# claforte/RayTracingWeekend.jl

Hardware: AMD Instinct MI355X
Metric: Msamples/s (pixels x spp) on scene_random_spheres 1920x1080 (higher is better)
Workload: dtype f32

## Files before the change

raytracingweekend.jl_amd/csrc/rtw_abi.hip:

```cpp
#include "rtw_host.hpp"
#include "rtw_kernels.hpp"

namespace rtwh {

__thread char g_err[512] = "";

bool test_aids() {
    static const bool on = [] { const char *e = getenv("RTW_ENABLE_TEST_AIDS"); return e != nullptr && atoi(e) != 0; }();
    return on;
}
const char *aid_env(const char *name) { return test_aids() ? getenv(name) : nullptr; }
bool aid_flag(const char *name) { const char *e = aid_env(name); return e != nullptr && atoi(e) != 0; }

int fail(int code, const char *fmt, ...) {
    va_list ap;
    va_start(ap, fmt);
    vsnprintf(g_err, sizeof g_err, fmt, ap);
    va_end(ap);
    return code;
}

std::mutex g_mu;
std::vector<CtxPtr> g_ctx;
std::atomic<unsigned> g_generation{1};
// ... 159 lines not shown
    *count = n;
    return 0;
}

const char *rtw_last_error(void) { return g_err; }

int rtw_scene_upload_f32(const rtw_scene_f32 *s, int device, rtw_scene_handle *out) { return upload_scene_f32(s, device, out); }
int rtw_scene_upload_f64(const rtw_scene_f64 *s, int device, rtw_scene_handle *out) { return upload_scene_f64(s, device, out); }

int rtw_scene_free(rtw_scene_handle h) {
    if (!h) return 0;
    DeviceGuard guard;
    HIP_IGNORE(hipSetDevice(h->device));
    void *ptrs[] = {h->geom, h->mat0, h->mat1, h->scan, h->mf_ops, h->c_mf_ops, h->c_mf_box, h->c_bound, h->c_exact, h->c_mat0, h->c_mat1, h->c_orig};
    for (void *q : ptrs) if (q) HIP_IGNORE(hipFree(q));
    delete h;
    return 0;
}

int rtw_render_device_f32(rtw_scene_handle s, const rtw_camera_f32 *c, const rtw_params *p, void *d_out, void *stream) {
    return render_device(s, c, p, d_out, stream);
}
int rtw_render_device_f64(rtw_scene_handle s, const rtw_camera_f64 *c, const rtw_params *p, void *d_out, void *stream) {
    return render_device(s, c, p, d_out, stream);
}
int rtw_render_f32(const rtw_scene_f32 *s, const rtw_camera_f32 *c, const rtw_params *p, float *out) {
    return render_host_f32(s, c, p, out);
}
int rtw_render_f64(const rtw_scene_f64 *s, const rtw_camera_f64 *c, const rtw_params *p, double *out) {
    return render_host_f64(s, c, p, out);
// ... 73 lines not shown
```

raytracingweekend.jl_amd/csrc/rtw_host.hpp:

```cpp
#pragma once
#pragma GCC visibility push(default)
#include "../../include/rtw_hip.h"
#pragma GCC visibility pop

#include <hip/hip_runtime.h>

#include <algorithm>
#include <atomic>
#include <cmath>
#include <cstdarg>
#include <cstdio>
#include <cstdlib>
#include <cstring>
#include <map>
#include <memory>
#include <mutex>
#include <string>
#include <thread>
#include <type_traits>
#include <vector>

#pragma GCC visibility push(hidden)

namespace rtw { struct DevCounters; }


struct rtw_scene_dev {
    int device;
    int is_f64;
    int n, n_pad;
    void *geom, *mat0, *mat1;
    void *scan;
    void *mf_ops;
    int mf_blocks;
    float mf_sc, mf_sigma2, mf_oo_keep, mf_o1_coef, mf_o_max;
    int n_huge, huge[2];
    void *c_mf_ops, *c_mf_box;
    float c_glo[3], c_ghi[3];
    int c_mf_blocks;
    float c_grid[6];
    int c_n_inlane, c_inlane[8];
    void *c_bound, *c_exact, *c_mat0, *c_mat1;
    unsigned short *c_orig;
    int c_groups_pad, c_big;
    double c_cs[3], c_rs;
    uint64_t content_hash;
};

namespace rtwh {

extern __thread char g_err[512];
// ... 146 lines not shown
```

raytracingweekend.jl_amd/csrc/rtw_kernels.hpp:

```cpp
#pragma once
#include "rtw_device.hpp"

namespace rtw {

#define RTW_JOB_PX 16
#ifndef RTW_SLOT_BYTES
#define RTW_SLOT_BYTES 4608
#endif
#define RTW_REF_BITS 9
#define RTW_REF_MASK 511u
#define RTW_SLOT_FREE 0xffffffffu
#define RTW_SLOT_OPENING 0xfffffffeu
#define RTW_SLOT_OPENING_BIT 0x80000000u
#define RTW_JOB_EOF 0xffffffffu
#define RTW_JOB_RETRY 0xfffffffeu

struct KParams {
    int width, height, spp, max_depth;
    uint64_t seed;
    int n_chunks;
    int chunk_spp;
    int shard_index, shard_count;
    int tiles_i, tiles_j;
    unsigned total_jobs;
// ... 345 lines not shown
    WgShared<T> *sh = reinterpret_cast<WgShared<T> *>(smem + list_bytes);
    constexpr size_t cell_bytes = MFMA ? mfma_cell_bytes<T>() : 0;
    V4 *lds_geom = reinterpret_cast<V4 *>(smem + list_bytes + shared_bytes + cell_bytes);
    WaveScratch ws = {nullptr, nullptr, nullptr};
    [[maybe_unused]] ulonglong2 *pool_rng = nullptr;
    [[maybe_unused]] unsigned long long pool_valid = 0;
    if constexpr (MFMA) {
        static_assert(list_bytes == 4 * RTW_PAIR_CAP * sizeof(unsigned), "the pair lists reuse the per-lane list area");
        const unsigned wv = threadIdx.x >> 6;
        unsigned char *cells = smem + list_bytes + shared_bytes;
        ws.pairs = reinterpret_cast<unsigned *>(smem) + wv * RTW_PAIR_CAP;
        ws.keys = reinterpret_cast<unsigned long long *>(cells) + wv * 64;
        ws.kidx = reinterpret_cast<unsigned *>(cells + 4 * 64 * sizeof(unsigned long long)) + wv * 64;
        pool_rng = reinterpret_cast<ulonglong2 *>(cells + mfma_cell_bytes<T>() - 4 * 64 * 16) + wv * 64;
    }
    unsigned short *lds_orig = reinterpret_cast<unsigned short *>(lds_geom + (CULL ? cull_exact_count(cull) : 0));
    [[maybe_unused]] unsigned *lds_tab = reinterpret_cast<unsigned *>(reinterpret_cast<unsigned char *>(lds_orig) + (CULL ? ((size_t)cull_exact_count(cull) * sizeof(unsigned short) + 15) / 16 * 16 : 0));
    if (threadIdx.x < P_arg.n_slots) { JobSlot *S0 = sh->slot(threadIdx.x, P_arg.slot_stride); S0->ready_seq = RTW_SLOT_FREE; S0->job = 0u; }
    if (threadIdx.x == 0) { sh->ticket = 0u; sh->eof = 0u; sh->fin_waves = 0u; sh->fin_segments = 0ull; sh->fin_samples = 0ull; sh->jobs.jc = 0ull; sh->jobs.jc_lock = 0u; sh->jobs.queue_off = 0u; sh->jobs.last_g = 0u; sh->jobs.static_used = 0u; sh->cam = cam_arg; sh->P = P_arg; }
    const KParams &P = sh->P;
    if (LDS_SCENE) {
        if (CULL) stage_cull_scene<T>(cull, lds_geom, lds_orig);
        else stage_scene<T>(scene, lds_geom);
        if constexpr (CULL && MFMA) {
            const unsigned *gt = reinterpret_cast<const unsigned *>(cull.mf_box + 8 * (cull.mf_blocks + 1));
            for (int i = threadIdx.x; i < cull_tab_words(cull.mf_blocks); i += blockDim.x) lds_tab[i] = gt[i];
        }
    }
    __syncthreads();

    if (lane == 0 && (threadIdx.x >> 6) < 4u) sh->t_wave[threadIdx.x >> 6] = wall_clock64();
    unsigned pool_next = 0, pool_end = 0;
    unsigned pool_slot = 0, pool_b = 0;
    bool have_ticket = false;
    unsigned tk_seq = 0, tk_b = 0;

    unsigned long long n_segments = 0, n_samples = 0;

// ... 12 lines not shown

    PhaseClock<PROFILE> clk;
    for (;;) {
        clk.start();
        T t_hit = 0;
        int idx = -1;
        if constexpr (MFMA && CULL) {
            if (__any(has_ray)) {
                MfmaCull mc = mfma_cull_of(cull);
                if (LDS_SCENE) mc.tab = lds_tab;
                if (LDS_SCENE) idx = hit_world_mfma<T>(scene, (const V4 *)lds_geom, ro, rd, has_ray, (T)1e-4, t_hit, ws, lane, clk, &mc, (const unsigned short *)lds_orig);
                else idx = hit_world_mfma<T>(scene, cull.exact, ro, rd, has_ray, (T)1e-4, t_hit, ws, lane, clk, &mc, cull.orig);
            }
        } else if constexpr (MFMA) {
            if (__any(has_ray)) {
                if (LDS_SCENE) idx = hit_world_mfma<T>(scene, (const V4 *)lds_geom, ro, rd, has_ray, (T)1e-4, t_hit, ws, lane, clk);
                else idx = hit_world_mfma<T>(scene, scene.geom, ro, rd, has_ray, (T)1e-4, t_hit, ws, lane, clk);
            }
        } else if (has_ray) {
            if (CULL && LDS_SCENE)
                idx = hit_world_cull<T, 256>(cull, (const V4 *)lds_geom, (const unsigned short *)lds_orig, ro, rd, (T)1e-4,
                                             (T)__builtin_huge_val(), t_hit, my_list, clk);
            else if (CULL)
                idx = hit_world_cull<T, 256>(cull, cull.exact, cull.orig, ro, rd, (T)1e-4, (T)__builtin_huge_val(), t_hit, my_list, clk);
            else if (LDS_SCENE)
                idx = hit_world<T, 256>(scene, (const V4 *)lds_geom, ro, rd, (T)1e-4, (T)__builtin_huge_val(), t_hit, my_list, clk);
            else
                idx = hit_world<T, 256>(scene, scene.geom, ro, rd, (T)1e-4, (T)__builtin_huge_val(), t_hit, my_list, clk);
        }
        n_segments += (unsigned long long)__popcll(__ballot(has_ray));
        clk.lap(2);
        if (PROFILE) { clk.count(8, 1u); clk.count(9, (unsigned)__popcll(__ballot(has_ray))); if (!__any(has_ray)) clk.count(10, 1u); }
// ... 311 lines not shown
```

raytracingweekend.jl_amd/csrc/rtw_launch.hip:

```cpp
#include "rtw_scene_view.hpp"
#include "rtw_kernels.hpp"
#include "rtw_instances.hpp"
#ifdef RTW_WITH_POOL
#include "rtw_pool.hpp"
#endif

namespace rtwh {

void make_udiv(unsigned d, unsigned *m, unsigned *s) {
    if (d <= 1) { *m = 0; *s = 0x80000000u; return; }
    unsigned l = 0;
    while ((1ull << l) < d) ++l;
    *m = (unsigned)((((1ull << l) - d) << 32) / d + 1);
    *s = l - 1;
}

template <typename T, typename CamT>
int launch_render(rtw_scene_handle scene, const CamT *cam, int n_views, const uint64_t *seeds, const rtw_params *p, void *d_out, hipStream_t stream,
                  RenderRec **rec_out, CtxPtr *ctx_out, const AccumPass *pass = nullptr) {
    if (!scene || !cam || (!d_out && !pass)) return fail(-1, "null argument");
    if (scene->is_f64 != (sizeof(T) == 8)) return fail(-4, "scene handle precision does not match the call");
    int nch, cs;
    if (int rc = validate_params(p, &nch, &cs)) return rc;
    if (pass) nch = pass->chunk_count;
// ... 43 lines not shown
    S.numerics = (p->flags & RTW_FLAG_NUMERICS_CONTRACT) ? rtw::NUM_CONTRACT : (p->flags & RTW_FLAG_NUMERICS_REFERENCE_FMA2) ? rtw::NUM_REFERENCE_FMA2 : rtw::NUM_REFERENCE;

    static const bool phase_profile = aid_env("RTW_PHASE_PROFILE") != nullptr;
    const size_t list_bytes = (size_t)RTW_LIST_CAP * 256 * sizeof(unsigned short);
    const size_t shared_bytes = (sizeof(rtw::WgShared<T>) + 15) / 16 * 16;
    const bool cull = (p->flags & RTW_FLAG_GROUP_CULL) != 0;
    rtw::CullScene<T> CS = cull_scene_of<T>(scene);
    CS.numerics = S.numerics;
    const size_t n_cull = (size_t)rtw::cull_exact_count(CS);
    static const bool force_valu = aid_env("RTW_SCAN") != nullptr && strcmp(aid_env("RTW_SCAN"), "valu") == 0;
    const bool mfma = (cull ? scene->c_mf_ops != nullptr : scene->mf_ops != nullptr) && !force_valu && !(p->flags & RTW_FLAG_SCAN_VALU);
    const size_t geom_bytes = cull ? n_cull * sizeof(V4) + ((n_cull * sizeof(unsigned short) + 15) / 16) * 16 +
                                         (mfma ? (size_t)rtw::cull_tab_words(scene->c_mf_blocks) * sizeof(unsigned) : 0)
                                   : (size_t)rtw::scene_geom_alloc(scene->n, scene->n_pad) * sizeof(V4);
    const bool lds_scene = geom_bytes <= RTW_LDS_SCENE_MAX_BYTES;
    const size_t lds_bytes = list_bytes + shared_bytes + (mfma ? rtw::mfma_cell_bytes<T>() : 0) + (lds_scene ? geom_bytes : 0);
    typedef void (*kern_t)(rtw::KParams, rtw::Camera<T>, rtw::DevScene<T>, rtw::CullScene<T>, T *, rtw::DevCounters *, rtw::BatchArgs<T>, rtw::AccumArgs);
    kern_t kern;
    if (cull && mfma && phase_profile) kern = lds_scene ? (kern_t)rtw::trace_kernel<T, true, true, true, true> : (kern_t)rtw::trace_kernel<T, false, false, true, true>;
    else if (cull && mfma) kern = lds_scene ? (kern_t)rtw::trace_kernel<T, false, true, true, true> : (kern_t)rtw::trace_kernel<T, false, false, true, true>;
    else if (cull && phase_profile) kern = lds_scene ? (kern_t)rtw::trace_kernel<T, true, true, true> : (kern_t)rtw::trace_kernel<T, false, false, true>;
    else if (cull) kern = lds_scene ? (kern_t)rtw::trace_kernel<T, false, true, true> : (kern_t)rtw::trace_kernel<T, false, false, true>;
    else if (mfma && phase_profile) kern = lds_scene ? (kern_t)rtw::trace_kernel<T, true, true, false, true> : (kern_t)rtw::trace_kernel<T, true, false, false, true>;
    else if (mfma) kern = lds_scene ? (kern_t)rtw::trace_kernel<T, false, true, false, true> : (kern_t)rtw::trace_kernel<T, false, false, false, true>;
    else if (phase_profile) kern = lds_scene ? (kern_t)rtw::trace_kernel<T, true, true, false> : (kern_t)rtw::trace_kernel<T, true, false, false>;
    else kern = lds_scene ? (kern_t)rtw::trace_kernel<T, false, true, false> : (kern_t)rtw::trace_kernel<T, false, false, false>;
    if (S.numerics == rtw::NUM_REFERENCE && lds_scene && mfma && !phase_profile)
        kern = cull ? (kern_t)rtw::trace_kernel<T, false, true, true, true, rtw::NUM_REFERENCE> : (kern_t)rtw::trace_kernel<T, false, true, false, true, rtw::NUM_REFERENCE>;
    const bool fixed = S.numerics == rtw::NUM_REFERENCE;
    if (batch && pass) kern = (kern_t)(sizeof(T) == 8 ? batch_accum_kernel_f64(cull, mfma, lds_scene, fixed, pass->adapt) : batch_accum_kernel_f32(cull, mfma, lds_scene, fixed, pass->adapt));
    else if (batch) kern = (kern_t)trace_instance_of<T, true, false, false>(cull, mfma, lds_scene, fixed);
// ... 101 lines not shown
        if (pass) {
            rtw::AccumView *hv = reinterpret_cast<rtw::AccumView *>(static_cast<char *>(rec->h_views) + cam_bytes + seed_bytes);
            for (int v = 0; v < n_views; ++v) { hv[v].words = pass->views[v].words; hv[v].samples = pass->views[v].samples; hv[v].pad = 0; }
            A.views = reinterpret_cast<const rtw::AccumView *>(static_cast<const char *>(rec->d_views) + cam_bytes + seed_bytes);
        }
        HIP_TRY(hipMemcpyAsync(rec->d_views, rec->h_views, bytes, hipMemcpyHostToDevice, stream));
        B.cams = reinterpret_cast<const rtw::Camera<T> *>(rec->d_views);
        B.seeds = reinterpret_cast<const unsigned long long *>(static_cast<const char *>(rec->d_views) + cam_bytes);
    }
    if (K.out_layout == 0 && p->shard_count > 1 && d_out)
        HIP_TRY(hipMemsetAsync(d_out, 0, (size_t)p->width * p->height * 3 * sizeof(T), stream));
    HIP_TRY(hipEventRecord(rec->ev0, stream));
    if (total_jobs > 0) {
        (void)hipGetLastError();
#ifdef RTW_WITH_POOL
        if (pool) hipLaunchKernelGGL(pool_kern, dim3((unsigned)grid), dim3((unsigned)block_threads), pool_lds, stream, K, C, S, (T *)d_out, rec->ctr);
        else
#endif
        hipLaunchKernelGGL(kern, dim3((unsigned)grid), dim3(256), lds_bytes, stream, K, C, S, CS, (T *)d_out, rec->ctr, B, A);
        HIP_TRY(hipGetLastError());
    }
    HIP_TRY(hipEventRecord(rec->ev1, stream));
    HIP_TRY(hipMemcpyAsync(rec->h_ctr, rec->ctr, rec->ctr_bytes, hipMemcpyDeviceToHost, stream));
    HIP_TRY(hipEventRecord(rec->ev2, stream));
    rec->used = true; rec->done = false;
    return 0;
}

int resolve_rec(RenderRec *r, rtw_stats_t *agg) {
    HIP_TRY(hipSetDevice(r->device));
    HIP_TRY(hipEventSynchronize(r->ev2));
// ... 82 lines not shown
```

raytracingweekend.jl_amd/csrc/rtw_scan.hpp:

```cpp
#pragma once
#include "rtw_path.hpp"

namespace rtw {

#define RTW_SPHERE_WORD 32
#define RTW_SPHERE_TAIL 8
__host__ __device__ inline int scene_geom_alloc(int n, int n_pad) {
    const int a = n_pad + RTW_SPHERE_TAIL, b = ((n + 31) / 32) * 32;
    return a > b ? a : b;
}
template <typename T> struct DevScene {
    const float *scan;
    const typename Vec4<T>::type *geom;
    const typename Vec4<T>::type *mat0;
    const typename Vec4<T>::type *mat1;
    int n, n_pad;
    const uint4 *mf_ops;
    int mf_blocks;
    float mf_sc;
    float mf_sigma2;
    float mf_oo_keep;
    float mf_o1_coef;
    float mf_o_max;
    int n_huge, huge[2];
    int numerics;
};

#define RTW_LIST_CAP 16
#define RTW_LDS_SCENE_MAX_BYTES (24 * 1024)

__device__ __forceinline__ uint32_t sign_word(float x) { return __float_as_uint(x); }
__device__ __forceinline__ uint32_t sign_word(double x) { return (uint32_t)((uint64_t)__double_as_longlong(x) >> 32); }

#ifndef RTW_SCAN_PRIO
#define RTW_SCAN_PRIO 1
#endif
template <typename T> struct ScanGroup;
template <> struct ScanGroup<float> { static constexpr int N = 4; };
template <> struct ScanGroup<double> { static constexpr int N = 4; };

// ... 164 lines not shown
```

raytracingweekend.jl_amd/csrc/rtw_scan_mfma.hpp:

```cpp
#pragma once
#include "rtw_scan.hpp"
#include "rtw_cull_tables.hpp"
#include "rtw_probes.hpp"

namespace rtw {

#define RTW_PAIR_CAP 512
typedef _Float16 rtw_h8 __attribute__((ext_vector_type(8)));
typedef float rtw_f16v __attribute__((ext_vector_type(16)));

__host__ __device__ inline int cull_tab_words(int blocks) { return ((blocks + 31) / 32 > 0 ? (blocks + 31) / 32 : 1) * RTW_CULL_TAB_WORDS; }
struct CullGrid {
    float inv[3], off[3];
};

struct MfmaCull {
    const uint4 *ops;
    const float *box;
    int blocks;
    float cs[3], rs;
    const void *mat0;
    float glo[3], ghi[3];
    int n_huge;
    int n_exact;
// ... 102 lines not shown
            }
            total += (unsigned)__popcll(act);
        }
    }
    __builtin_amdgcn_wave_barrier();
    test_singles<T, WITH_R>(num, src, rad, o, d, tmin, ws, singles, total, lane, orig, prof, sink);
    __builtin_amdgcn_wave_barrier();
}

template <typename T, typename SRC, typename RAD, typename ORIG = NoOrig, typename SINK = NoSink>
__device__ __forceinline__ void resolve_pairs(int num, SRC src, RAD rad, V3<T> o, V3<T> d, T tmin, const WaveScratch &ws, unsigned n, unsigned lane, ORIG orig = ORIG(), unsigned *prof = nullptr, SINK sink = SINK()) {
    if (num == NUM_REFERENCE_FMA2) resolve_pairs_impl<T, true>(num, src, rad(), o, d, tmin, ws, n, lane, orig, prof, sink);
    else resolve_pairs_impl<T, false>(num, src, nullptr, o, d, tmin, ws, n, lane, orig, prof, sink);
}

template <typename T, typename SRC, typename ORIG = NoOrig, typename CLK = NoClock, typename SINK = NoSink>
__device__ __forceinline__ int hit_world_mfma(const DevScene<T> &w, SRC src, V3<T> o, V3<T> d, bool has_ray, T tmin, T &t_hit,
                                              const WaveScratch &ws, unsigned lane, CLK &&clk = NoClock(),
                                              const MfmaCull *mc = nullptr, ORIG orig = ORIG(), SINK sink = SINK()) {
    constexpr bool CULLED = !__is_same(ORIG, NoOrig);
    auto rad = [&]() -> const typename Vec4<T>::type * { if constexpr (CULLED) return (const typename Vec4<T>::type *)mc->mat0; else return w.mat0; };
    const float ox = (float)o.x, oy = (float)o.y, oz = (float)o.z, dx = (float)d.x, dy = (float)d.y, dz = (float)d.z;
    const float s2 = __builtin_fmaf(dz, dz, __builtin_fmaf(dy, dy, dx * dx));
    const float oinf = __builtin_fmaxf(__builtin_fmaxf(__builtin_fabsf(ox), __builtin_fabsf(oy)), __builtin_fabsf(oz));
    const bool ok = has_ray && s2 <= 1.0009f && oinf <= w.mf_o_max;
    if constexpr (SINK::on()) { if (has_ray) sink.ray(lane, ok, w.mf_sc); }
    const float q = __builtin_fmaf(oz, dz, __builtin_fmaf(oy, dy, ox * dx));
    const float oo = __builtin_fmaf(oz, oz, __builtin_fmaf(oy, oy, ox * ox));
    const float o1 = (__builtin_fabsf(ox) + __builtin_fabsf(oy)) + __builtin_fabsf(oz);
    const float oop = __builtin_fmaf(oo, w.mf_oo_keep, -(w.mf_o1_coef * o1));
    const float tq = w.mf_sigma2 * __builtin_fmaf(q, q, -oop);
    const float z = ok ? 1.0f : 0.0f, z2 = z + z, zs2 = z2 * w.mf_sc;
    const float fp[3] = {__builtin_fmaf(-q, dx, ox) * zs2, __builtin_fmaf(-q, dy, oy) * zs2, __builtin_fmaf(-q, dz, oz) * zs2};
    const float dx2 = dx * z2, dy2 = dy * z2, dz2 = dz * z2;
    const float fq[6] = {dx2 * dx, dy2 * dy, dz2 * dz, (dx2 + dx2) * dy, (dx2 + dx2) * dz, (dy2 + dy2) * dz};
// ... 80 lines not shown
        B1[0] = __builtin_bit_cast(rtw_h8, q10); B1[1] = __builtin_bit_cast(rtw_h8, q11);
        B2[0] = __builtin_bit_cast(rtw_h8, q20); B2[1] = __builtin_bit_cast(rtw_h8, q21);
    }
    const unsigned lane_const = lane << 16;
    unsigned total = 0;
    {
        unsigned long long key0 = ~0ull;
        [[maybe_unused]] unsigned kidx0 = 0u;
        using V4 = typename Vec4<T>::type;
        const int n_huge = CULLED ? (RTW_INLANE_FILTER ? mc->n_exact : mc->n_huge) : w.n_huge;
        for (int hgi = 0; hgi < n_huge; ++hgi) {
            int si;
            if constexpr (CULLED) si = __builtin_amdgcn_readfirstlane((int)mc->tab[6 * RTW_CULL_BINS + 4 + hgi]);
            else si = hgi == 0 ? w.huge[0] : w.huge[1];
            const V4 sg = src[si];
            if constexpr (SINK::on()) { if (has_ray) { if constexpr (CULLED) sink.inlane(lane, (int)orig[si]); else sink.inlane(lane, si); } }
            T hb_, disc_, root_ = 0;
            T rr_ = T(0);
            if (w.numerics == NUM_REFERENCE_FMA2) rr_ = rad()[si].x;
            sphere_disc<T>(w.numerics, sg.x, sg.y, sg.z, sg.w, rr_, o, d, hb_, disc_);
            if (has_ray && sphere_root<T>(hb_, disc_, tmin, (T)__builtin_huge_val(), root_)) {
                unsigned tie = (unsigned)si;
                if constexpr (CULLED) tie = ((unsigned)orig[si] << 16) | (unsigned)si;
                if constexpr (sizeof(T) == 4) {
                    const unsigned low = CULLED ? ((0xffffu - (tie >> 16)) << 16) | (tie & 0xffffu) : 0xffffffffu - tie;
                    const unsigned long long k = ((unsigned long long)__float_as_uint((float)root_) << 32) | (unsigned long long)low;
                    key0 = k < key0 ? k : key0;
                } else {
                    const unsigned long long tb = (unsigned long long)__double_as_longlong((double)root_);
                    if (tb < key0 || (tb == key0 && tie + 1u > kidx0)) { key0 = tb; kidx0 = tie + 1u; }
                }
            }
        }
        if constexpr (sizeof(T) == 4) ws.keys[lane] = key0;
        else { ws.keys[lane] = key0; ws.kidx[lane] = kidx0; }
    }
    if constexpr (CULLED && RTW_INLANE_FILTER) {
        using V4 = typename Vec4<T>::type;
        for (int hgi = mc->n_exact; hgi < mc->n_huge; ++hgi) {
            const int si = __builtin_amdgcn_readfirstlane((int)mc->tab[6 * RTW_CULL_BINS + 4 + hgi]);
// ... 124 lines not shown
        if (m != 0u) {
            const unsigned pos = __builtin_amdgcn_mbcnt_hi((unsigned)(act >> 32), __builtin_amdgcn_mbcnt_lo((unsigned)act, total));
            reinterpret_cast<uint2 *>(ws.pairs)[pos] = uint2{m, lane_const + (unsigned)cur * 32u};
        }
        total += (unsigned)__popcll(act);
        clk.lap(4);
    }
    }
    if (use_prio) __builtin_amdgcn_s_setprio(sizeof(T) == 4 ? 1 : 0);
    { unsigned pr[3] = {0u, 0u, 0u}; resolve_pairs<T>(w.numerics, src, rad, o, d, tmin, ws, total, lane, orig, clk.on() ? pr : nullptr, sink); clk.count(13, total); clk.count(14, pr[0]); clk.count(15, pr[1]); clk.count(28, pr[2]); }
    RTW_PROBE_RESOLVE_TWICE();
    clk.lap(5);
    int idx;
    if constexpr (sizeof(T) == 4) {
        const unsigned long long k = ws.keys[lane];
        idx = k == ~0ull ? -1 : (CULLED ? (int)((unsigned)k & 0xffffu) : (int)(0xffffffffu - (unsigned)k));
        t_hit = __uint_as_float((unsigned)(k >> 32));
    } else {
        const unsigned long long k = ws.keys[lane];
        const unsigned ki = ws.kidx[lane];
        idx = ki == 0u ? -1 : (CULLED ? (int)((ki - 1u) & 0xffffu) : (int)ki - 1);
        t_hit = __longlong_as_double((long long)k);
    }
    if (!has_ray) idx = -1;
    return idx;
}

}
```

raytracingweekend.jl_amd/csrc/rtw_scene.hip:

```cpp
#include "rtw_scene_view.hpp"
#include "rtw_cull_tables.hpp"

namespace rtwh {

template <typename SceneT>
void kd_split(const SceneT *s, std::vector<int> &ids, int lo, int hi, std::vector<std::vector<int>> &groups) {
    const int cnt = hi - lo;
    if (cnt <= RTW_CULL_GS) {
        if (cnt > 0) groups.emplace_back(ids.begin() + lo, ids.begin() + hi);
        return;
    }
    double mn[3] = {1e300, 1e300, 1e300}, mx[3] = {-1e300, -1e300, -1e300};
    for (int k = lo; k < hi; ++k) {
        const double c[3] = {(double)s->cx[ids[k]], (double)s->cy[ids[k]], (double)s->cz[ids[k]]};
        for (int a = 0; a < 3; ++a) { mn[a] = std::min(mn[a], c[a]); mx[a] = std::max(mx[a], c[a]); }
    }
    int ax = 0;
    for (int a = 1; a < 3; ++a) if (mx[a] - mn[a] > mx[ax] - mn[ax]) ax = a;
    const int unit = cnt > 2 * RTW_CULL_GS ? 2 * RTW_CULL_GS : RTW_CULL_GS;
    int half = ((cnt / 2 + unit - 1) / unit) * unit;
    if (half >= cnt) half = cnt - 1;
    auto key = [&](int i) { return ax == 0 ? (double)s->cx[i] : ax == 1 ? (double)s->cy[i] : (double)s->cz[i]; };
    std::nth_element(ids.begin() + lo, ids.begin() + lo + half, ids.begin() + hi, [&](int a, int b) { return key(a) < key(b); });
    kd_split(s, ids, lo, lo + half, groups);
    kd_split(s, ids, lo + half, hi, groups);
}

template <typename T, typename V4, typename SceneT>
void material_rows(const SceneT *s, int i, V4 &m0, V4 &m1) {
    m0 = V4{s->r[i], s->param[i], (T)s->kind[i], (T)0};
    m1 = V4{s->ar[i], s->ag[i], s->ab[i], (T)0};
    if (s->kind[i] == rtw::DIELECTRIC) {
        const rtw::DielConst<T> c = rtw::dielectric_constants<T>(s->param[i]);
        m0.w = c.inv_ir;
        m1 = V4{c.r0_front, c.r0_back, (T)0, (T)0};
    }
}

template <typename T, typename V4>
int build_mfma_operands(const std::vector<V4> &geom, int n, rtw_scene_dev *h, void **ops_out, int *blocks_out, int n_skip = 0, const int *skip = nullptr);

template <typename T, typename SceneT>
int build_cull(const SceneT *s, rtw_scene_dev *h) {
    using V4 = typename rtw::Vec4<T>::type;
    const int n = s->n;
    constexpr int pair = 2 * RTW_CULL_BG, GS = RTW_CULL_GS;
    std::vector<int> small_ids, big_ids;
    if (n > 0) {
        std::vector<double> rr(n);
        for (int i = 0; i < n; ++i) rr[i] = std::fabs((double)s->r[i]);
        std::vector<double> tmp(rr);
        std::nth_element(tmp.begin(), tmp.begin() + (n - 1) / 2, tmp.end());
        const double thr = 4.0 * tmp[(n - 1) / 2];
        for (int i = 0; i < n; ++i) (rr[i] > thr ? big_ids : small_ids).push_back(i);
    }
// ... 110 lines not shown
            for (int a = 0; a < 3; ++a) { h->c_glo[a] = std::min(h->c_glo[a], q[a]); h->c_ghi[a] = std::max(h->c_ghi[a], q[4 + a]); }
        }
        CullTables ct;
        build_cull_tables(bx.data(), nb, h->c_glo, h->c_ghi, h->c_n_inlane, h->c_inlane, &ct);
        for (int k = 0; k < 3; ++k) { h->c_grid[k] = ct.inv[k]; h->c_grid[3 + k] = ct.off[k]; }
        std::vector<float> cells(ct.words.size(), 0.0f);
        memcpy(cells.data(), ct.words.data(), ct.words.size() * sizeof(unsigned));
        bx.insert(bx.end(), cells.begin(), cells.end());
        HIP_TRY(hipMalloc(&h->c_mf_box, bx.size() * sizeof(float)));
        HIP_TRY(hipMemcpy(h->c_mf_box, bx.data(), bx.size() * sizeof(float), hipMemcpyHostToDevice));
    }
    return 0;
}

template <typename T, typename V4>
int build_mfma_operands(const std::vector<V4> &geom, int n, rtw_scene_dev *h, void **ops_out, int *blocks_out, int n_skip, const int *skip) {
    *ops_out = nullptr; *blocks_out = 0;
    if (n <= 0) return 0;
    auto live = [&](int i) { return i < n && (double)geom[i].w > -1e29; };
    auto in_filter = [&](int i) { if (!live(i)) return false; for (int k = 0; k < n_skip; ++k) if (skip[k] == i) return false; return true; };
    double emax = 0;
    for (int i = 0; i < n; ++i) {
        if (!live(i)) continue;
        const double r = std::sqrt(std::fabs((double)geom[i].w));
        emax = std::max(emax, std::max(std::max(std::fabs((double)(float)geom[i].x), std::fabs((double)(float)geom[i].y)),
                                       std::max(std::fabs((double)(float)geom[i].z), r)));
    }
    if (!(emax > 0) || !std::isfinite(emax)) return 0;
    int ex = 0;
    (void)std::frexp(emax, &ex);
    if (ex > 40 || ex < -40) return 0;
    const double sc = std::ldexp(1.0, 8 - ex), sig2 = sc * sc;
    const double phi_c = std::ldexp(1.0, -25) / sc, phi_k = std::ldexp(1.0, -20) / sig2;
    const double A_S = std::ldexp(1.0, -17), A_r = std::ldexp(12.0, -22);
    auto split = [](double x, unsigned &p1, unsigned &p2) {
        const float xf = (float)x;
        const _Float16 h1 = (_Float16)xf;
        const _Float16 h2 = (_Float16)(xf - (float)h1);
        unsigned short b1, b2;
        memcpy(&b1, &h1, 2); memcpy(&b2, &h2, 2);
        p1 = b1; p2 = b2;
    };
    const int nb = (n + 31) / 32;
    std::vector<uint4> ops((size_t)(nb + 1) * 128);
    for (int blk = 0; blk <= nb; ++blk)
        for (int lane = 0; lane < 64; ++lane) {
            const int i = lane & 31, H = lane >> 5;
            const int sph = blk * 32 + 16 * ((i >> 2) & 1) + (((i >> 3) << 2) | (i & 3));
            double fq[6] = {0, 0, 0, 0, 0, 0}, fl[3] = {0, 0, 0};
            double kx = -1073741824.0;
            if (in_filter(sph)) {
                const double cx = (double)(float)geom[sph].x, cy = (double)(float)geom[sph].y, cz = (double)(float)geom[sph].z;
                const double r2 = (double)geom[sph].w, c2 = cx * cx + cy * cy + cz * cz;
                const double Gs = 1.02 * ((2 * A_S + A_r) * c2 + A_r * r2 + 9 * phi_c * (std::fabs(cx) + std::fabs(cy) + std::fabs(cz)) + 1.5 * phi_k);
                kx = (r2 - c2 + Gs) * sig2;
                const double hs = 0.5 * sig2;
                fq[0] = cx * cx * hs; fq[1] = cy * cy * hs; fq[2] = cz * cz * hs; fq[3] = cx * cy * hs; fq[4] = cx * cz * hs; fq[5] = cy * cz * hs;
                fl[0] = cx * sc; fl[1] = cy * sc; fl[2] = cz * sc;
// ... 18 lines not shown
            }
            ops[(size_t)blk * 128 + lane] = m1;
            ops[(size_t)blk * 128 + 64 + lane] = m2;
        }
    HIP_TRY(hipMalloc(ops_out, ops.size() * sizeof(uint4)));
    HIP_TRY(hipMemcpy(*ops_out, ops.data(), ops.size() * sizeof(uint4), hipMemcpyHostToDevice));
    *blocks_out = nb;
    h->mf_sc = (float)sc; h->mf_sigma2 = (float)sig2;
    float keep = (float)(1.0 - 1.02 * 2 * A_S);
    if ((double)keep > 1.0 - 1.02 * 2 * A_S) keep = std::nextafter(keep, 0.0f);
    h->mf_oo_keep = keep;
    float coef = (float)(1.02 * 9 * phi_c);
    if ((double)coef < 1.02 * 9 * phi_c) coef = std::nextafter(coef, INFINITY);
    h->mf_o1_coef = coef;
    h->mf_o_max = (float)(std::ldexp(1.0, 13) / sc);
    return 0;
}

template <typename T, typename SceneT>
int upload_scene(const SceneT *s, int device, rtw_scene_handle *out) {
    if (!s || !out) return fail(-1, "null argument");
    if (s->n < 0) return fail(-2, "scene.n < 0");
    if (s->n > 0 && (!s->cx || !s->cy || !s->cz || !s->r || !s->kind || !s->ar || !s->ag || !s->ab || !s->param))
        return fail(-1, "null scene array");
    for (int i = 0; i < s->n; ++i) {
        if (s->kind[i] < 0 || s->kind[i] > 2) return fail(-3, "sphere %d: unknown material kind %d", i, s->kind[i]);
        if (!std::isfinite((double)s->cx[i]) || !std::isfinite((double)s->cy[i]) || !std::isfinite((double)s->cz[i]) ||
            !std::isfinite((double)s->r[i]))
            return fail(-3, "sphere %d: centre / radius is not finite", i);
    }
// ... 65 lines not shown
        const double med = sorted[n / 2];
        for (int pick = 0; pick < 2; ++pick) {
            int best = -1;
            for (int i = 0; i < n; ++i) {
                if (!(ra[i] >= 16.0 * med) || !std::isfinite(ra[i])) continue;
                if (h->n_huge > 0 && h->huge[0] == i) continue;
                if (best < 0 || ra[i] > ra[best]) best = i;
            }
            if (best < 0) break;
            h->huge[h->n_huge++] = best;
        }
    }
    static const bool env_no_huge = aid_flag("RTW_NO_HUGE");
    if (env_no_huge) h->n_huge = 0;
    if (int rc = build_mfma_operands<T>(geom, n, h.get(), &h->mf_ops, &h->mf_blocks, h->n_huge, h->huge)) return rc;
    if (int rc = build_cull<T>(s, h.get())) return rc;
    *out = h.release();
    return 0;
}

int upload_scene_f32(const rtw_scene_f32 *s, int device, rtw_scene_handle *out) { return upload_scene<float>(s, device, out); }
int upload_scene_f64(const rtw_scene_f64 *s, int device, rtw_scene_handle *out) { return upload_scene<double>(s, device, out); }

}
```

raytracingweekend.jl_amd/csrc/rtw_scene_view.hpp:

```cpp
#pragma once
#include "rtw_host.hpp"
#include "rtw_device.hpp"

namespace rtwh {

template <typename T>
rtw::CullScene<T> cull_scene_of(const rtw_scene_dev *h) {
    using V4 = typename rtw::Vec4<T>::type;
    rtw::CullScene<T> C;
    C.box = (const T *)h->c_bound; C.exact = (const V4 *)h->c_exact; C.orig = h->c_orig;
    C.mat0 = (const V4 *)h->c_mat0; C.mat1 = (const V4 *)h->c_mat1;
    C.n_groups_pad = h->c_groups_pad; C.n_big = h->c_big;
    C.cs[0] = (T)h->c_cs[0]; C.cs[1] = (T)h->c_cs[1]; C.cs[2] = (T)h->c_cs[2]; C.rs = (T)h->c_rs;
    C.kappa = sizeof(T) == 4 ? (T)0.00390625 : (T)2.384185791015625e-07;
    C.mf_ops = (const uint4 *)h->c_mf_ops; C.mf_box = (const float *)h->c_mf_box; C.mf_blocks = h->c_mf_blocks;
    for (int k = 0; k < 3; ++k) { C.mf_glo[k] = h->c_glo[k]; C.mf_ghi[k] = h->c_ghi[k]; }
    static_assert(RTW_CULL_INLANE_MAX == 8, "rtw_scene_dev::c_inlane");
    C.n_huge = h->c_mf_ops ? h->c_n_inlane : 0;
    C.n_huge_exact = h->c_mf_ops ? std::min(h->n_huge, h->c_n_inlane) : 0;
    for (int k = 0; k < 3; ++k) { C.grid.inv[k] = h->c_grid[k]; C.grid.off[k] = h->c_grid[3 + k]; }
    C.numerics = rtw::NUM_REFERENCE;
    return C;
}

template <typename T>
rtw::DevScene<T> dev_scene_of(const rtw_scene_dev *h) {
    using V4 = typename rtw::Vec4<T>::type;
    rtw::DevScene<T> S;
    memset(&S, 0, sizeof S);
    S.geom = (const V4 *)h->geom; S.mat0 = (const V4 *)h->mat0; S.mat1 = (const V4 *)h->mat1;
    S.scan = (const float *)(h->scan ? h->scan : h->geom);
    S.n = h->n; S.n_pad = h->n_pad;
    S.mf_ops = (const uint4 *)h->mf_ops; S.mf_blocks = h->mf_blocks;
    S.mf_sc = h->mf_sc; S.mf_sigma2 = h->mf_sigma2; S.mf_oo_keep = h->mf_oo_keep; S.mf_o1_coef = h->mf_o1_coef; S.mf_o_max = h->mf_o_max;
    S.n_huge = h->mf_ops ? h->n_huge : 0; S.huge[0] = h->huge[0]; S.huge[1] = h->huge[1];
    return S;
}

}
```

Before: 5827.

## Reorder spheres into spatially coherent blocks for the plain MFMA scan

At upload, the spheres are partitioned by median splits along the widest axis into blocks of 32, so each MFMA operand block holds spatially nearby spheres. A second set of geometry, material and MFMA operand arrays is built in that order, plus an index map back to the caller's original sphere order. The plain (non-cull) MFMA kernel reads these arrays and uses the map to break ties consistently. The likely intent is tighter per-block bounds, giving better block rejection and locality. The cost is extra device memory, an extra LDS array of indices, and tie-break work in the hit loop.

```diff
diff --git a/raytracingweekend.jl_amd/csrc/rtw_abi.hip b/raytracingweekend.jl_amd/csrc/rtw_abi.hip
--- a/raytracingweekend.jl_amd/csrc/rtw_abi.hip
+++ b/raytracingweekend.jl_amd/csrc/rtw_abi.hip
@@ -197,6 +197,8 @@
     HIP_IGNORE(hipSetDevice(h->device));
     void *ptrs[] = {h->geom, h->mat0, h->mat1, h->scan, h->mf_ops, h->c_mf_ops, h->c_mf_box, h->c_bound, h->c_exact, h->c_mat0, h->c_mat1, h->c_orig};
     for (void *q : ptrs) if (q) HIP_IGNORE(hipFree(q));
+    if (h->p_orig) HIP_IGNORE(hipFree(h->p_orig));
+    if (!h->p_alias) for (void *q : {h->p_mf_ops, h->p_geom, h->p_mat0, h->p_mat1}) if (q) HIP_IGNORE(hipFree(q));
     delete h;
     return 0;
 }
diff --git a/raytracingweekend.jl_amd/csrc/rtw_host.hpp b/raytracingweekend.jl_amd/csrc/rtw_host.hpp
--- a/raytracingweekend.jl_amd/csrc/rtw_host.hpp
+++ b/raytracingweekend.jl_amd/csrc/rtw_host.hpp
@@ -35,6 +35,9 @@
     int mf_blocks;
     float mf_sc, mf_sigma2, mf_oo_keep, mf_o1_coef, mf_o_max;
     int n_huge, huge[2];
+    void *p_mf_ops, *p_geom, *p_mat0, *p_mat1;
+    unsigned short *p_orig;
+    int p_alias, p_n, p_n_pad, p_mf_blocks, p_huge[2];
     void *c_mf_ops, *c_mf_box;
     float c_glo[3], c_ghi[3];
     int c_mf_blocks;
diff --git a/raytracingweekend.jl_amd/csrc/rtw_kernels.hpp b/raytracingweekend.jl_amd/csrc/rtw_kernels.hpp
--- a/raytracingweekend.jl_amd/csrc/rtw_kernels.hpp
+++ b/raytracingweekend.jl_amd/csrc/rtw_kernels.hpp
@@ -383,7 +383,7 @@
         ws.kidx = reinterpret_cast<unsigned *>(cells + 4 * 64 * sizeof(unsigned long long)) + wv * 64;
         pool_rng = reinterpret_cast<ulonglong2 *>(cells + mfma_cell_bytes<T>() - 4 * 64 * 16) + wv * 64;
     }
-    unsigned short *lds_orig = reinterpret_cast<unsigned short *>(lds_geom + (CULL ? cull_exact_count(cull) : 0));
+    unsigned short *lds_orig = reinterpret_cast<unsigned short *>(lds_geom + (CULL ? cull_exact_count(cull) : MFMA ? scene_geom_alloc(scene.n, scene.n_pad) : 0));
     [[maybe_unused]] unsigned *lds_tab = reinterpret_cast<unsigned *>(reinterpret_cast<unsigned char *>(lds_orig) + (CULL ? ((size_t)cull_exact_count(cull) * sizeof(unsigned short) + 15) / 16 * 16 : 0));
     if (threadIdx.x < P_arg.n_slots) { JobSlot *S0 = sh->slot(threadIdx.x, P_arg.slot_stride); S0->ready_seq = RTW_SLOT_FREE; S0->job = 0u; }
     if (threadIdx.x == 0) { sh->ticket = 0u; sh->eof = 0u; sh->fin_waves = 0u; sh->fin_segments = 0ull; sh->fin_samples = 0ull; sh->jobs.jc = 0ull; sh->jobs.jc_lock = 0u; sh->jobs.queue_off = 0u; sh->jobs.last_g = 0u; sh->jobs.static_used = 0u; sh->cam = cam_arg; sh->P = P_arg; }
@@ -391,6 +391,7 @@
     if (LDS_SCENE) {
         if (CULL) stage_cull_scene<T>(cull, lds_geom, lds_orig);
         else stage_scene<T>(scene, lds_geom);
+        if constexpr (!CULL && MFMA) { for (int i = threadIdx.x; i < scene_geom_alloc(scene.n, scene.n_pad); i += blockDim.x) lds_orig[i] = scene.orig[i]; }
         if constexpr (CULL && MFMA) {
             const unsigned *gt = reinterpret_cast<const unsigned *>(cull.mf_box + 8 * (cull.mf_blocks + 1));
             for (int i = threadIdx.x; i < cull_tab_words(cull.mf_blocks); i += blockDim.x) lds_tab[i] = gt[i];
@@ -433,8 +434,8 @@
             }
         } else if constexpr (MFMA) {
             if (__any(has_ray)) {
-                if (LDS_SCENE) idx = hit_world_mfma<T>(scene, (const V4 *)lds_geom, ro, rd, has_ray, (T)1e-4, t_hit, ws, lane, clk);
-                else idx = hit_world_mfma<T>(scene, scene.geom, ro, rd, has_ray, (T)1e-4, t_hit, ws, lane, clk);
+                if (LDS_SCENE) idx = hit_world_mfma<T, const V4 *, const unsigned short *, PhaseClock<PROFILE> &, NoSink, false>(scene, (const V4 *)lds_geom, ro, rd, has_ray, (T)1e-4, t_hit, ws, lane, clk, nullptr, (const unsigned short *)lds_orig);
+                else idx = hit_world_mfma<T, const V4 *, const unsigned short *, PhaseClock<PROFILE> &, NoSink, false>(scene, scene.geom, ro, rd, has_ray, (T)1e-4, t_hit, ws, lane, clk, nullptr, scene.orig);
             }
         } else if (has_ray) {
             if (CULL && LDS_SCENE)
diff --git a/raytracingweekend.jl_amd/csrc/rtw_launch.hip b/raytracingweekend.jl_amd/csrc/rtw_launch.hip
--- a/raytracingweekend.jl_amd/csrc/rtw_launch.hip
+++ b/raytracingweekend.jl_amd/csrc/rtw_launch.hip
@@ -81,7 +81,18 @@
                                          (mfma ? (size_t)rtw::cull_tab_words(scene->c_mf_blocks) * sizeof(unsigned) : 0)
                                    : (size_t)rtw::scene_geom_alloc(scene->n, scene->n_pad) * sizeof(V4);
     const bool lds_scene = geom_bytes <= RTW_LDS_SCENE_MAX_BYTES;
-    const size_t lds_bytes = list_bytes + shared_bytes + (mfma ? rtw::mfma_cell_bytes<T>() : 0) + (lds_scene ? geom_bytes : 0);
+    const bool plain_order = mfma && !cull;
+    [[maybe_unused]] const rtw::DevScene<T> S_caller = S;
+    size_t plain_bytes = 0;
+    if (plain_order) {
+        if (!scene->p_mf_ops || !scene->p_orig) return fail(-9, "internal: the scene has no arrays in the plain scan's order");
+        const int num = S.numerics;
+        S = dev_scene_plain_of<T>(scene);
+        S.numerics = num;
+        const size_t na = (size_t)rtw::scene_geom_alloc(S.n, S.n_pad);
+        plain_bytes = na * sizeof(V4) + ((na * sizeof(unsigned short) + 15) / 16) * 16;
+    }
+    const size_t lds_bytes = list_bytes + shared_bytes + (mfma ? rtw::mfma_cell_bytes<T>() : 0) + (lds_scene ? (plain_order ? plain_bytes : geom_bytes) : 0);
     typedef void (*kern_t)(rtw::KParams, rtw::Camera<T>, rtw::DevScene<T>, rtw::CullScene<T>, T *, rtw::DevCounters *, rtw::BatchArgs<T>, rtw::AccumArgs);
     kern_t kern;
     if (cull && mfma && phase_profile) kern = lds_scene ? (kern_t)rtw::trace_kernel<T, true, true, true, true> : (kern_t)rtw::trace_kernel<T, false, false, true, true>;
@@ -213,7 +224,7 @@
     if (total_jobs > 0) {
         (void)hipGetLastError();
 #ifdef RTW_WITH_POOL
-        if (pool) hipLaunchKernelGGL(pool_kern, dim3((unsigned)grid), dim3((unsigned)block_threads), pool_lds, stream, K, C, S, (T *)d_out, rec->ctr);
+        if (pool) hipLaunchKernelGGL(pool_kern, dim3((unsigned)grid), dim3((unsigned)block_threads), pool_lds, stream, K, C, S_caller, (T *)d_out, rec->ctr);
         else
 #endif
         hipLaunchKernelGGL(kern, dim3((unsigned)grid), dim3(256), lds_bytes, stream, K, C, S, CS, (T *)d_out, rec->ctr, B, A);
diff --git a/raytracingweekend.jl_amd/csrc/rtw_plain_layout.hpp b/raytracingweekend.jl_amd/csrc/rtw_plain_layout.hpp
--- /dev/null
+++ b/raytracingweekend.jl_amd/csrc/rtw_plain_layout.hpp
@@ -0,0 +1,54 @@
+#pragma once
+#include <algorithm>
+#include <vector>
+
+#define RTW_PLAIN_BLOCK 32
+
+namespace rtwh {
+
+struct PlainLayout {
+    int blocks = 0;
+    std::vector<int> slot;
+};
+
+inline void build_plain_layout(const double *cx, const double *cy, const double *cz, int n, PlainLayout *out) {
+    constexpr int B = RTW_PLAIN_BLOCK;
+    out->blocks = n > 0 ? (n + B - 1) / B : 0;
+    out->slot.assign((size_t)out->blocks * B, -1);
+    if (out->blocks <= 1) {
+        for (int i = 0; i < n; ++i) out->slot[i] = i;
+        return;
+    }
+    std::vector<int> ids(n);
+    for (int i = 0; i < n; ++i) ids[i] = i;
+    const double *c[3] = {cx, cy, cz};
+    struct Node { int lo, hi, leaf0, leaves; };
+    std::vector<Node> todo;
+    todo.push_back(Node{0, n, 0, out->blocks});
+    while (!todo.empty()) {
+        const Node nd = todo.back();
+        todo.pop_back();
+        const int cnt = nd.hi - nd.lo;
+        if (nd.leaves == 1) {
+            std::sort(ids.begin() + nd.lo, ids.begin() + nd.hi);
+            for (int k = 0; k < cnt; ++k) out->slot[(size_t)nd.leaf0 * B + k] = ids[nd.lo + k];
+            continue;
+        }
+        int ax = 0;
+        double ext[3];
+        for (int a = 0; a < 3; ++a) {
+            double mn = c[a][ids[nd.lo]], mx = mn;
+            for (int k = nd.lo + 1; k < nd.hi; ++k) { mn = std::min(mn, c[a][ids[k]]); mx = std::max(mx, c[a][ids[k]]); }
+            ext[a] = mx - mn;
+        }
+        for (int a = 1; a < 3; ++a) if (ext[a] > ext[ax]) ax = a;
+        const double *key = c[ax];
+        std::sort(ids.begin() + nd.lo, ids.begin() + nd.hi, [key](int a, int b) { return key[a] < key[b] || (key[a] == key[b] && a < b); });
+        const int base = cnt / nd.leaves, rem = cnt % nd.leaves, left = nd.leaves / 2;
+        const int left_cnt = left * base + std::min(rem, left);
+        todo.push_back(Node{nd.lo, nd.lo + left_cnt, nd.leaf0, left});
+        todo.push_back(Node{nd.lo + left_cnt, nd.hi, nd.leaf0 + left, nd.leaves - left});
+    }
+}
+
+}
diff --git a/raytracingweekend.jl_amd/csrc/rtw_scan.hpp b/raytracingweekend.jl_amd/csrc/rtw_scan.hpp
--- a/raytracingweekend.jl_amd/csrc/rtw_scan.hpp
+++ b/raytracingweekend.jl_amd/csrc/rtw_scan.hpp
@@ -24,6 +24,7 @@
     float mf_o_max;
     int n_huge, huge[2];
     int numerics;
+    const unsigned short *orig;
 };
 
 #define RTW_LIST_CAP 16
diff --git a/raytracingweekend.jl_amd/csrc/rtw_scan_mfma.hpp b/raytracingweekend.jl_amd/csrc/rtw_scan_mfma.hpp
--- a/raytracingweekend.jl_amd/csrc/rtw_scan_mfma.hpp
+++ b/raytracingweekend.jl_amd/csrc/rtw_scan_mfma.hpp
@@ -140,11 +140,13 @@
     else resolve_pairs_impl<T, false>(num, src, nullptr, o, d, tmin, ws, n, lane, orig, prof, sink);
 }
 
-template <typename T, typename SRC, typename ORIG = NoOrig, typename CLK = NoClock, typename SINK = NoSink>
+template <typename T, typename SRC, typename ORIG = NoOrig, typename CLK = NoClock, typename SINK = NoSink, bool VOTE = !__is_same(ORIG, NoOrig)>
 __device__ __forceinline__ int hit_world_mfma(const DevScene<T> &w, SRC src, V3<T> o, V3<T> d, bool has_ray, T tmin, T &t_hit,
                                               const WaveScratch &ws, unsigned lane, CLK &&clk = NoClock(),
                                               const MfmaCull *mc = nullptr, ORIG orig = ORIG(), SINK sink = SINK()) {
-    constexpr bool CULLED = !__is_same(ORIG, NoOrig);
+    constexpr bool HAS_ORIG = !__is_same(ORIG, NoOrig);
+    constexpr bool CULLED = VOTE;
+    static_assert(HAS_ORIG || !VOTE, "the group cull's order comes with its index array");
     auto rad = [&]() -> const typename Vec4<T>::type * { if constexpr (CULLED) return (const typename Vec4<T>::type *)mc->mat0; else return w.mat0; };
     const float ox = (float)o.x, oy = (float)o.y, oz = (float)o.z, dx = (float)d.x, dy = (float)d.y, dz = (float)d.z;
     const float s2 = __builtin_fmaf(dz, dz, __builtin_fmaf(dy, dy, dx * dx));
@@ -255,16 +257,16 @@
             if constexpr (CULLED) si = __builtin_amdgcn_readfirstlane((int)mc->tab[6 * RTW_CULL_BINS + 4 + hgi]);
             else si = hgi == 0 ? w.huge[0] : w.huge[1];
             const V4 sg = src[si];
-            if constexpr (SINK::on()) { if (has_ray) { if constexpr (CULLED) sink.inlane(lane, (int)orig[si]); else sink.inlane(lane, si); } }
+            if constexpr (SINK::on()) { if (has_ray) { if constexpr (HAS_ORIG) sink.inlane(lane, (int)orig[si]); else sink.inlane(lane, si); } }
             T hb_, disc_, root_ = 0;
             T rr_ = T(0);
             if (w.numerics == NUM_REFERENCE_FMA2) rr_ = rad()[si].x;
             sphere_disc<T>(w.numerics, sg.x, sg.y, sg.z, sg.w, rr_, o, d, hb_, disc_);
             if (has_ray && sphere_root<T>(hb_, disc_, tmin, (T)__builtin_huge_val(), root_)) {
                 unsigned tie = (unsigned)si;
-                if constexpr (CULLED) tie = ((unsigned)orig[si] << 16) | (unsigned)si;
+                if constexpr (HAS_ORIG) tie = ((unsigned)orig[si] << 16) | (unsigned)si;
                 if constexpr (sizeof(T) == 4) {
-                    const unsigned low = CULLED ? ((0xffffu - (tie >> 16)) << 16) | (tie & 0xffffu) : 0xffffffffu - tie;
+                    const unsigned low = HAS_ORIG ? ((0xffffu - (tie >> 16)) << 16) | (tie & 0xffffu) : 0xffffffffu - tie;
                     const unsigned long long k = ((unsigned long long)__float_as_uint((float)root_) << 32) | (unsigned long long)low;
                     key0 = k < key0 ? k : key0;
                 } else {
@@ -419,12 +421,12 @@
     int idx;
     if constexpr (sizeof(T) == 4) {
         const unsigned long long k = ws.keys[lane];
-        idx = k == ~0ull ? -1 : (CULLED ? (int)((unsigned)k & 0xffffu) : (int)(0xffffffffu - (unsigned)k));
+        idx = k == ~0ull ? -1 : (HAS_ORIG ? (int)((unsigned)k & 0xffffu) : (int)(0xffffffffu - (unsigned)k));
         t_hit = __uint_as_float((unsigned)(k >> 32));
     } else {
         const unsigned long long k = ws.keys[lane];
         const unsigned ki = ws.kidx[lane];
-        idx = ki == 0u ? -1 : (CULLED ? (int)((ki - 1u) & 0xffffu) : (int)ki - 1);
+        idx = ki == 0u ? -1 : (HAS_ORIG ? (int)((ki - 1u) & 0xffffu) : (int)ki - 1);
         t_hit = __longlong_as_double((long long)k);
     }
     if (!has_ray) idx = -1;
diff --git a/raytracingweekend.jl_amd/csrc/rtw_scene.hip b/raytracingweekend.jl_amd/csrc/rtw_scene.hip
--- a/raytracingweekend.jl_amd/csrc/rtw_scene.hip
+++ b/raytracingweekend.jl_amd/csrc/rtw_scene.hip
@@ -1,5 +1,6 @@
 #include "rtw_scene_view.hpp"
 #include "rtw_cull_tables.hpp"
+#include "rtw_plain_layout.hpp"
 
 namespace rtwh {
 
@@ -38,7 +39,7 @@
 }
 
 template <typename T, typename V4>
-int build_mfma_operands(const std::vector<V4> &geom, int n, rtw_scene_dev *h, void **ops_out, int *blocks_out, int n_skip = 0, const int *skip = nullptr);
+int build_mfma_operands(const std::vector<V4> &geom, int n, rtw_scene_dev *h, void **ops_out, int *blocks_out, int n_skip = 0, const int *skip = nullptr, int n_rows = -1);
 
 template <typename T, typename SceneT>
 int build_cull(const SceneT *s, rtw_scene_dev *h) {
@@ -179,11 +180,12 @@
 }
 
 template <typename T, typename V4>
-int build_mfma_operands(const std::vector<V4> &geom, int n, rtw_scene_dev *h, void **ops_out, int *blocks_out, int n_skip, const int *skip) {
+int build_mfma_operands(const std::vector<V4> &geom, int n, rtw_scene_dev *h, void **ops_out, int *blocks_out, int n_skip, const int *skip, int n_rows) {
     *ops_out = nullptr; *blocks_out = 0;
     if (n <= 0) return 0;
     auto live = [&](int i) { return i < n && (double)geom[i].w > -1e29; };
-    auto in_filter = [&](int i) { if (!live(i)) return false; for (int k = 0; k < n_skip; ++k) if (skip[k] == i) return false; return true; };
+    if (n_rows < 0) n_rows = n;
+    auto in_filter = [&](int i) { if (!live(i) || i >= n_rows) return false; for (int k = 0; k < n_skip; ++k) if (skip[k] == i) return false; return true; };
     double emax = 0;
     for (int i = 0; i < n; ++i) {
         if (!live(i)) continue;
@@ -206,7 +208,7 @@
         memcpy(&b1, &h1, 2); memcpy(&b2, &h2, 2);
         p1 = b1; p2 = b2;
     };
-    const int nb = (n + 31) / 32;
+    const int nb = (n_rows + 31) / 32;
     std::vector<uint4> ops((size_t)(nb + 1) * 128);
     for (int blk = 0; blk <= nb; ++blk)
         for (int lane = 0; lane < 64; ++lane) {
@@ -255,6 +257,55 @@
     if ((double)coef < 1.02 * 9 * phi_c) coef = std::nextafter(coef, INFINITY);
     h->mf_o1_coef = coef;
     h->mf_o_max = (float)(std::ldexp(1.0, 13) / sc);
+    return 0;
+}
+
+template <typename T, typename V4>
+int build_plain(const std::vector<V4> &geom, const std::vector<V4> &mat0, const std::vector<V4> &mat1, int n, rtw_scene_dev *h) {
+    if (!h->mf_ops) return 0;
+    static const bool keep_env = aid_env("RTW_PLAIN_ORDER") != nullptr && strcmp(aid_env("RTW_PLAIN_ORDER"), "caller") == 0;
+    auto is_huge = [&](int i) { for (int k = 0; k < h->n_huge; ++k) if (h->huge[k] == i) return true; return false; };
+    std::vector<int> filt;
+    std::vector<double> cx, cy, cz;
+    for (int i = 0; i < n; ++i) {
+        if (is_huge(i)) continue;
+        filt.push_back(i);
+        cx.push_back((double)geom[i].x); cy.push_back((double)geom[i].y); cz.push_back((double)geom[i].z);
+    }
+    PlainLayout L;
+    build_plain_layout(cx.data(), cy.data(), cz.data(), (int)filt.size(), &L);
+    constexpr int grp = rtw::ScanGroup<T>::N;
+    const int n_rows = L.blocks * RTW_PLAIN_BLOCK, np = n_rows + h->n_huge, np_pad = ((np + grp - 1) / grp) * grp;
+    const int np_alloc = rtw::scene_geom_alloc(np, np_pad);
+    std::vector<unsigned short> orig;
+    if (keep_env || L.blocks <= 1 || np_alloc >= 65536) {
+        h->p_alias = 1;
+        h->p_mf_ops = h->mf_ops; h->p_geom = h->geom; h->p_mat0 = h->mat0; h->p_mat1 = h->mat1;
+        h->p_n = n; h->p_n_pad = h->n_pad; h->p_mf_blocks = h->mf_blocks; h->p_huge[0] = h->huge[0]; h->p_huge[1] = h->huge[1];
+        orig.resize((size_t)rtw::scene_geom_alloc(n, h->n_pad));
+        for (size_t i = 0; i < orig.size(); ++i) orig[i] = (unsigned short)i;
+    } else {
+        std::vector<V4> g(np_alloc, V4{(T)0, (T)0, (T)0, (T)-1e30}), m0(np_alloc, V4{(T)1, (T)0, (T)0, (T)0}), m1(np_alloc, V4{(T)0, (T)0, (T)0, (T)0});
+        orig.assign((size_t)np_alloc, 0);
+        auto put = [&](int k, int i) { g[k] = geom[i]; m0[k] = mat0[i]; m1[k] = mat1[i]; orig[k] = (unsigned short)i; };
+        for (int k = 0; k < n_rows; ++k) if (L.slot[k] >= 0) put(k, filt[L.slot[k]]);
+        for (int k = 0; k < h->n_huge; ++k) { put(n_rows + k, h->huge[k]); h->p_huge[k] = n_rows + k; }
+        h->p_n = np; h->p_n_pad = np_pad;
+        const size_t bytes = sizeof(V4) * (size_t)np_alloc;
+        HIP_TRY(hipMalloc(&h->p_geom, bytes));
+        HIP_TRY(hipMalloc(&h->p_mat0, bytes));
+        HIP_TRY(hipMalloc(&h->p_mat1, bytes));
+        HIP_TRY(hipMemcpy(h->p_geom, g.data(), bytes, hipMemcpyHostToDevice));
+        HIP_TRY(hipMemcpy(h->p_mat0, m0.data(), bytes, hipMemcpyHostToDevice));
+        HIP_TRY(hipMemcpy(h->p_mat1, m1.data(), bytes, hipMemcpyHostToDevice));
+        if (int rc = build_mfma_operands<T>(g, np, h, &h->p_mf_ops, &h->p_mf_blocks, h->n_huge, h->p_huge, n_rows)) return rc;
+        if (!h->p_mf_ops) return fail(-9, "internal: no matrix-pipe operands for the plain scan's order");
+    }
+    if (aid_env("RTW_DEBUG"))
+        fprintf(stderr, "[rtw debug] plain scan layout: %d spheres through the filter, %d blocks, %s\n", (int)filt.size(), h->p_mf_blocks,
+                h->p_alias ? "the caller's order" : "its own order");
+    HIP_TRY(hipMalloc((void **)&h->p_orig, orig.size() * sizeof(unsigned short)));
+    HIP_TRY(hipMemcpy(h->p_orig, orig.data(), orig.size() * sizeof(unsigned short), hipMemcpyHostToDevice));
     return 0;
 }
 
@@ -350,6 +401,7 @@
     static const bool env_no_huge = aid_flag("RTW_NO_HUGE");
     if (env_no_huge) h->n_huge = 0;
     if (int rc = build_mfma_operands<T>(geom, n, h.get(), &h->mf_ops, &h->mf_blocks, h->n_huge, h->huge)) return rc;
+    if (int rc = build_plain<T>(geom, mat0, mat1, n, h.get())) return rc;
     if (int rc = build_cull<T>(s, h.get())) return rc;
     *out = h.release();
     return 0;
diff --git a/raytracingweekend.jl_amd/csrc/rtw_scene_view.hpp b/raytracingweekend.jl_amd/csrc/rtw_scene_view.hpp
--- a/raytracingweekend.jl_amd/csrc/rtw_scene_view.hpp
+++ b/raytracingweekend.jl_amd/csrc/rtw_scene_view.hpp
@@ -37,4 +37,16 @@
     return S;
 }
 
+template <typename T>
+rtw::DevScene<T> dev_scene_plain_of(const rtw_scene_dev *h) {
+    using V4 = typename rtw::Vec4<T>::type;
+    rtw::DevScene<T> S = dev_scene_of<T>(h);
+    S.geom = (const V4 *)h->p_geom; S.mat0 = (const V4 *)h->p_mat0; S.mat1 = (const V4 *)h->p_mat1;
+    S.n = h->p_n; S.n_pad = h->p_n_pad;
+    S.mf_ops = (const uint4 *)h->p_mf_ops; S.mf_blocks = h->p_mf_blocks;
+    S.huge[0] = h->p_huge[0]; S.huge[1] = h->p_huge[1];
+    S.orig = h->p_orig;
+    return S;
 }
+
+}
```

Result: faster. 5894 (median of 6 runs) (+1.2%).
